# heheyas/V3D

Hardware: AMD Instinct MI355X
Metric: multi-view frames/sec, V3D_512 18-frame 25-step EDM (higher is better)
Workload: dtype bf16; 1 GPU; BASELINE.json configs[1]: V3D_512 random-init SVD-XT weights, 1x18x4x64x64 latent, 25 EulerEDM steps, cfg 4.5 (LinearPredictionGuider), 18-frame VideoDecoder decode to 512x512, one sample per GPU; frames=18, edm_steps=25, parallelism=replica x1, hip_graph=False

## Files before the change

include/v3d_hip.h:

```cpp
#ifndef V3D_HIP_H
#define V3D_HIP_H

#include <stdint.h>

#ifdef __cplusplus
extern "C" {
#endif

#define V3D_ABI_VERSION 9

typedef void* v3d_stream_t;

enum {
    V3D_OK = 0,
    V3D_ERR_ARG = -1,
    V3D_ERR_LAUNCH = -2,
};

int v3d_abi_version(void);
const char* v3d_last_error(void);
int v3d_device_info(int32_t* out4);

enum { V3D_GEMM_LINEAR = 0, V3D_GEMM_CONV3X3 = 1, V3D_GEMM_CONVT3 = 2 };

// ... 32 lines not shown
    const void* A2;
    int64_t K1, lda2;
} v3d_gemm_args;

int v3d_gemm(const v3d_gemm_args* args, v3d_stream_t stream);
int v3d_gemm_gn_in_supported(const v3d_gemm_args* args);

int v3d_ff_fused(const void* x, int64_t ldx, const void* W1p, const float* b1, const void* W2p, const float* b2,
                 const void* res1, int64_t ldr1, const void* res2, int64_t ldr2, const float* coef, int64_t coef_rpg,
                 float c_acc, float c_res1, float c_res2, void* out, int64_t ldo, int64_t M, int32_t C, int32_t hidden,
                 v3d_stream_t stream);

int v3d_ln_ff_fused(const void* x, int64_t ldx, float ln_eps, const void* W1p, const float* b1, const void* W2p, const float* b2,
                 const void* res1, int64_t ldr1, const void* res2, int64_t ldr2, const float* coef, int64_t coef_rpg,
                 float c_acc, float c_res1, float c_res2, void* out, int64_t ldo, int64_t M, int32_t C, int32_t hidden,
                 v3d_stream_t stream);
int v3d_ln_proj(const void* x, int64_t ldx, float eps, const void* Wp, const float* bias, void* out, int64_t ldo, void* outT,
                int64_t M, int32_t C, int32_t N, int32_t n_rm, int64_t S, v3d_stream_t stream);
int v3d_sizeof_gemm_args(void);

int v3d_groupnorm_stats(const void* x1, int64_t C1, const void* x2, int64_t C2, float* stats, int64_t nslots,
                        int64_t n_img, int64_t S, int32_t groups, int64_t imgs_per_stat, v3d_stream_t stream);
int v3d_groupnorm_stats_table(const void* x1, int64_t C1, const void* x2, int64_t C2, float* stats, int64_t nslots, uint32_t* tickets,
                              int64_t n_img, int64_t S, int32_t groups, int64_t imgs_per_stat, const float* gamma, const float* beta,
                              double count, float eps, float* table, v3d_stream_t stream);
int v3d_groupnorm_finalize(const float* stats, int64_t nslots, double* sums, int64_t n_stat, int32_t groups,
                           const float* gamma, const float* beta, int64_t C, double count, float eps, float* table,
                           v3d_stream_t stream);
int v3d_groupnorm_apply(const void* x1, int64_t C1, const void* x2, int64_t C2, const float* table, void* out,
                        int64_t n_img, int64_t S, int64_t imgs_per_stat, int32_t silu, v3d_stream_t stream);

// ... 103 lines not shown
```

v3d_amd/csrc/ff.hip:

```cpp
#include "common.h"

namespace {

struct FFP {
    const bf16_t* x;
    const bf16_t* W1;
    const bf16_t* W2;
    const float* b1;
    const float* b2;
    const bf16_t* res1;
    const bf16_t* res2;
    const float* coef;
    bf16_t* out;
    long long M, ldx, ldr1, ldr2, ldo, coef_rpg;
    float c_acc, c_res1, c_res2;
    int hidden;
    float ln_eps;
    unsigned w1_bytes, w2_bytes;
};

template <int I, int N, typename F>
__device__ __forceinline__ void ff_static_for(F&& f) {
    if constexpr (I < N) {
        f(std::integral_constant<int, I>{});
        ff_static_for<I + 1, N>(f);
    }
}

template <int NMFMA, int NVALU>
__device__ __forceinline__ void ff_tick_pipeline() {
    __builtin_amdgcn_sched_group_barrier(0x100, 8, 0);
    ff_static_for<0, NMFMA>([&](auto ic) __attribute__((always_inline)) {
        constexpr int i = decltype(ic)::value;
        __builtin_amdgcn_sched_group_barrier(0x008, 1, 0);
        __builtin_amdgcn_sched_group_barrier(0x100, 1, 0);
        if constexpr (i % 4 == 1) {
            __builtin_amdgcn_sched_group_barrier(0x004, 2, 0);
            __builtin_amdgcn_sched_group_barrier(0x020, 1, 0);
        }
        __builtin_amdgcn_sched_group_barrier(0x402, NVALU, 0);
    });
}

__device__ __forceinline__ int ff_swz(int row) { return (0x78 >> (((row >> 2) & 3) * 2)) & 3; }

template <int C, bool LN>
__global__ __launch_bounds__(256, 1) void ff_fused_kernel(FFP p) {
    constexpr int NT = C / 32;
    constexpr int NK = C / 16;
    constexpr int NO = C / 32;
    constexpr int W1_STAGE = 64 * 64;
    constexpr int W1_BYTES = NT * W1_STAGE;
    constexpr int W2_BYTES = C * 64;
    constexpr int NP1 = NT * 4, NP2 = C / 16;
    static_assert(NP1 % 4 == 0 && NP2 % 4 == 0, "pieces per wave");
    constexpr int PPW1 = NP1 / 4, PPW2 = NP2 / 4;
    constexpr int SROW = 128 + 16;
    constexpr int STAGE_REGION = 32 * SROW;
    static_assert(NO % 2 == 0, "staging geometry");
    constexpr int RING = 2 * W1_BYTES + 3 * W2_BYTES;
    constexpr int B2_OFF = RING + 4 * STAGE_REGION;
    constexpr int LDS_BYTES = B2_OFF + C * 4;
// ... 18 lines not shown
    const long long nblocks = p.M / 128;

    f32x16 acc2[NO];
#pragma unroll
    for (int o = 0; o < NO; ++o)
#pragma unroll
        for (int r = 0; r < 16; ++r) acc2[o][r] = 0.f;
    f32x16 sA[2][2];
    bf16x8 hh[2][2];
    bf16x8 xr[NK];

    auto load_x = [&](long long blk) __attribute__((always_inline)) {
        const bf16_t* xz = p.x + (blk * 128 + wave * 32 + l31) * p.ldx + hi * 8;
#pragma unroll
        for (int k = 0; k < NK; ++k) xr[k] = *reinterpret_cast<const bf16x8*>(xz + k * 16);
    };

    constexpr int NPD = 4;
    bf16x8 wf[NPD];
    int w2_wr_slot = 0, w2_rd_slot = 0;
    auto tick = [&](auto pa_c, auto pg_c, auto pb_c, auto pd_c, auto d2_c, int j) __attribute__((always_inline)) {
        constexpr int PA = decltype(pa_c)::value, PG = decltype(pg_c)::value, PB = decltype(pb_c)::value, PDM = decltype(pd_c)::value;
        constexpr bool D2 = decltype(d2_c)::value != 0;
        constexpr int NB = PB >= 0 ? 2 * NO : 0, NA = PA >= 0 ? 4 * NT : 0, NS = 2 * NO + 4 * NT;
        float4 bu[4], bv[4];
        const unsigned char* bz = reinterpret_cast<const unsigned char*>(p.b1 + (j == nslab ? 0 : j + 1) * 64 + hi * 4);
        if constexpr (PA >= 0) {
#pragma unroll
            for (int g = 0; g < 4; ++g) {
                bu[g] = *reinterpret_cast<const float4*>(bz + g * 32);
// ... 119 lines not shown
    ff_static_for<0, 2 * PPW1>([&](auto ic) __attribute__((always_inline)) {
        constexpr int k = decltype(ic)::value % PPW1, par = decltype(ic)::value / PPW1;
        __builtin_amdgcn_raw_ptr_buffer_load_lds(rsW1, (__attribute__((address_space(3))) void*)(w1ring + par * W1_BYTES + k * W1_STAGE + wave * 1024), 16,
                                                 (int)voff1, par * 64 * C * 2 + k * 4096, 0, 0);
    });
    ld1 = 2;
    ff_static_for<0, PPW2>([&](auto ic) __attribute__((always_inline)) {
        constexpr int k = decltype(ic)::value;
        __builtin_amdgcn_raw_ptr_buffer_load_lds(rsW2, (__attribute__((address_space(3))) void*)(w2ring + (wave + 4 * k) * 1024), 16, (int)voff2,
                                                 k * w2_step, 0, 0);
    });
    ld2 = 1;
    w2_wr_slot = 1;
    load_x(blk);
    asm volatile("s_waitcnt vmcnt(0)" ::: "memory");
    if constexpr (LN) ln_rows_inplace<NK>(xr, p.ln_eps);
    __builtin_amdgcn_s_barrier();
    tick(I0{}, IX{}, IX{}, IX{}, I0{}, -1);

    u32x4 r1[2][4];
    u32x2 r2[2][8];
    auto fetch_res = [&](long long mw0_, int ps, u32x4 (&q1)[4], u32x2 (&q2)[8]) __attribute__((always_inline)) {
        int lane_e = lane;
        asm volatile("" : "+v"(lane_e));
        if (p.res1) {
            const bf16_t* rz = p.res1 + mw0_ * p.ldr1 + ps * 64;
#pragma unroll
            for (int it = 0; it < 4; ++it) {
                const int c = it * 64 + lane_e;
                q1[it] = *reinterpret_cast<const u32x4*>(rz + (long long)(c >> 3) * p.ldr1 + (c & 7) * 8);
// ... 10 lines not shown
#pragma unroll
            for (int k = 0; k < 8; ++k) q2[k] = u32x2{0, 0};
        }
    };

    while (true) {
        const long long mw0 = blk * 128 + wave * 32;
        tick(I1{}, I0{}, IX{}, I0{}, I1{}, 0);
        for (int j = 1; j + 2 < nslab; j += 2) {
            tick(I0{}, I1{}, I0{}, I1{}, I1{}, j);
            tick(I1{}, I0{}, I1{}, I0{}, I1{}, j + 1);
        }
        const long long nxt = blk + gridDim.x;
        load_x(nxt < nblocks ? nxt : blk);
        tick(IX{}, I1{}, I0{}, I1{}, I0{}, nslab - 1);
        if constexpr (LN) ln_rows_inplace<NK>(xr, p.ln_eps);
        fetch_res(mw0, 0, r1[0], r2[0]);
        tick(I0{}, IX{}, I1{}, IX{}, I1{}, nslab);

        {
            int lane_e = lane;
            asm volatile("" : "+v"(lane_e));
            const int l31 = lane_e & 31, hi = lane_e >> 5, lane = lane_e;
            const long long m = mw0 + l31;
            float ca = p.c_acc, c1 = p.c_res1, c2 = p.c_res2;
            if (p.coef) {
                const float* cf = p.coef + (m / p.coef_rpg) * 3;
                ca = cf[0]; c1 = cf[1]; c2 = cf[2];
            }
#pragma unroll
            for (int ps = 0; ps < NO / 2; ++ps) {
                const int col0 = ps * 64;
                if (ps + 1 < NO / 2) fetch_res(mw0, ps + 1, r1[(ps + 1) & 1], r2[(ps + 1) & 1]);
                if (p.res1) {
#pragma unroll
                    for (int it = 0; it < 4; ++it) {
                        const int c = it * 64 + lane;
                        *reinterpret_cast<u32x4*>(stage + (c >> 3) * SROW + (c & 7) * 16) = r1[ps & 1][it];
                    }
                    asm volatile("s_waitcnt lgkmcnt(0)" ::: "memory");
                }
#pragma unroll
                for (int oo = 0; oo < 2; ++oo) {
                    const int o = ps * 2 + oo;
#pragma unroll
                    for (int g = 0; g < 4; ++g) {
                        const int ch = oo * 32 + g * 8 + hi * 4;
                        const float4 b = *reinterpret_cast<const float4*>(lds + B2_OFF + (col0 + ch) * 4);
                        float v[4] = {ca * (acc2[o][4 * g + 0] + b.x), ca * (acc2[o][4 * g + 1] + b.y), ca * (acc2[o][4 * g + 2] + b.z),
                                      ca * (acc2[o][4 * g + 3] + b.w)};
                        if (p.res1) {
                            const uint2 rr = *reinterpret_cast<const uint2*>(stage + l31 * SROW + ch * 2);
                            v[0] += c1 * bflo(rr.x); v[1] += c1 * bfhi(rr.x); v[2] += c1 * bflo(rr.y); v[3] += c1 * bfhi(rr.y);
                        }
                        if (p.res2) {
                            const u32x2 rr = r2[ps & 1][oo * 4 + g];
                            v[0] += c2 * bflo(rr.x); v[1] += c2 * bfhi(rr.x); v[2] += c2 * bflo(rr.y); v[3] += c2 * bfhi(rr.y);
                        }
                        *reinterpret_cast<uint2*>(stage + l31 * SROW + ch * 2) = make_uint2(pack2bf(v[0], v[1]), pack2bf(v[2], v[3]));
                    }
#pragma unroll
                    for (int r = 0; r < 16; ++r) acc2[o][r] = 0.f;
                }
                asm volatile("s_waitcnt lgkmcnt(0)" ::: "memory");
                bf16_t* oz = p.out + mw0 * p.ldo + col0;
#pragma unroll
                for (int c0 = 0; c0 < 256; c0 += 64) {
// ... 2 lines not shown
                        *reinterpret_cast<const uint4*>(stage + (c >> 3) * SROW + (c & 7) * 16);
                }
            }
        }
        if (nxt >= nblocks) break;
        blk = nxt;
    }
    asm volatile("s_waitcnt vmcnt(0)" ::: "memory");
}

}

static int ff_fused_launch(const void* x, int64_t ldx, float ln_eps, const void* W1p, const float* b1, const void* W2p, const float* b2,
                           const void* res1, int64_t ldr1, const void* res2, int64_t ldr2, const float* coef, int64_t coef_rpg,
                           float c_acc, float c_res1, float c_res2, void* out, int64_t ldo, int64_t M, int32_t C, int32_t hidden,
                           v3d_stream_t stream) {
    V3D_REQUIRE(x && W1p && b1 && W2p && b2 && out, "v3d_ff_fused: null pointer");
    V3D_REQUIRE(C == 320, "v3d_ff_fused: built for C = 320 (got %d); wider levels use the two-GEMM path", C);
    V3D_REQUIRE(hidden >= 128 && hidden % 64 == 0 && hidden * (long long)C * 4 < (1ll << 31), "v3d_ff_fused: bad hidden size %d", hidden);
    V3D_REQUIRE(M > 0 && M % 128 == 0, "v3d_ff_fused: M must be a multiple of 128 (got %lld)", (long long)M);
    V3D_REQUIRE(ldx % 8 == 0 && ldo % 8 == 0 && (!res1 || ldr1 % 8 == 0) && (!res2 || ldr2 % 4 == 0), "v3d_ff_fused: row strides");
    V3D_REQUIRE(((((uintptr_t)x | (uintptr_t)W1p | (uintptr_t)W2p | (uintptr_t)out | (uintptr_t)b1 | (uintptr_t)b2) & 15) == 0) &&
                    (!res1 || ((uintptr_t)res1 & 15) == 0) && (!res2 || ((uintptr_t)res2 & 7) == 0),
                "v3d_ff_fused: misaligned pointer");
    V3D_REQUIRE(!coef || coef_rpg > 0, "v3d_ff_fused: coef_rpg must be > 0");
    FFP p;
    p.x = (const bf16_t*)x; p.W1 = (const bf16_t*)W1p; p.W2 = (const bf16_t*)W2p; p.b1 = b1; p.b2 = b2;
    p.res1 = (const bf16_t*)res1; p.res2 = (const bf16_t*)res2; p.coef = coef; p.out = (bf16_t*)out;
    p.M = M; p.ldx = ldx; p.ldr1 = ldr1; p.ldr2 = ldr2; p.ldo = ldo; p.coef_rpg = coef_rpg;
    p.c_acc = c_acc; p.c_res1 = c_res1; p.c_res2 = c_res2; p.hidden = hidden; p.ln_eps = ln_eps;
    p.w1_bytes = (unsigned)(2ll * hidden * C * 2);
    p.w2_bytes = (unsigned)((long long)C * hidden * 2);
    const long long nblocks = M / 128;
    const int grid = (int)(nblocks < v3d_num_cus() ? nblocks : v3d_num_cus());
    if (ln_eps > 0.f)
        hipLaunchKernelGGL((ff_fused_kernel<320, true>), dim3(grid), dim3(256), 0, (hipStream_t)stream, p);
    else
        hipLaunchKernelGGL((ff_fused_kernel<320, false>), dim3(grid), dim3(256), 0, (hipStream_t)stream, p);
    return v3d_check_launch("v3d_ff_fused");
}

extern "C" int v3d_ff_fused(const void* x, int64_t ldx, const void* W1p, const float* b1, const void* W2p, const float* b2,
                            const void* res1, int64_t ldr1, const void* res2, int64_t ldr2, const float* coef, int64_t coef_rpg,
                            float c_acc, float c_res1, float c_res2, void* out, int64_t ldo, int64_t M, int32_t C, int32_t hidden,
                            v3d_stream_t stream) {
    return ff_fused_launch(x, ldx, 0.f, W1p, b1, W2p, b2, res1, ldr1, res2, ldr2, coef, coef_rpg, c_acc, c_res1, c_res2, out, ldo, M, C, hidden, stream);
}

extern "C" int v3d_ln_ff_fused(const void* x, int64_t ldx, float ln_eps, const void* W1p, const float* b1, const void* W2p, const float* b2,
                               const void* res1, int64_t ldr1, const void* res2, int64_t ldr2, const float* coef, int64_t coef_rpg,
                               float c_acc, float c_res1, float c_res2, void* out, int64_t ldo, int64_t M, int32_t C, int32_t hidden,
                               v3d_stream_t stream) {
    V3D_REQUIRE(ln_eps > 0.f, "v3d_ln_ff_fused: ln_eps must be > 0");
    return ff_fused_launch(x, ldx, ln_eps, W1p, b1, W2p, b2, res1, ldr1, res2, ldr2, coef, coef_rpg, c_acc, c_res1, c_res2, out, ldo, M, C, hidden, stream);
}
```

v3d_amd/csrc/norm.hip:

```cpp

#include "common.h"

namespace {

constexpr int NVMAX = 2;
constexpr int CMAX = 4096;

struct GNGeom {
    int VC;
    int TPR;
    int RPP;
    int NV;
};

__host__ __device__ inline GNGeom gn_geom(long long C) {
    GNGeom g;
    g.VC = (int)(C / 8);
    g.TPR = g.VC < 256 ? g.VC : 256;
    g.RPP = 256 / g.TPR;
    g.NV = (g.VC + g.TPR - 1) / g.TPR;
    return g;
}

__device__ __forceinline__ uint4 load_vec2(const bf16_t* x1, long long C1, const bf16_t* x2, long long C2, long long row, int c) {
// ... 171 lines not shown
            }
        }
#pragma unroll
        for (int j = 0; j < NV; ++j) {
            const int v = tcol + j * g.TPR;
            if (v < g.VC) {
#pragma unroll
                for (int e = 0; e < 8; ++e) {
                    sh_s[(long long)trow * C + v * 8 + e] = s[j][e];
                    sh_q[(long long)trow * C + v * 8 + e] = q[j][e];
                }
            }
        }
    }
    __syncthreads();
    const int cpg = (int)(C / groups);
    if (tid < groups) {
        float a = 0.f, b = 0.f;
        for (int r = 0; r < g.RPP; ++r)
            for (int c = tid * cpg; c < (tid + 1) * cpg; ++c) {
                a += sh_s[(long long)r * C + c];
                b += sh_q[(long long)r * C + c];
            }
        const long long slot = (img % imgs_per_stat) * gridDim.x + blockIdx.x;
        float* dst = stats + (((img / imgs_per_stat) * nslots + slot) * groups + tid) * 2;
        if constexpr (FUSE) {
            const f32x2_t v = {a, b};
            asm volatile("global_store_dwordx2 %0, %1, off sc0 sc1\n\ts_waitcnt vmcnt(0)" ::"v"(dst), "v"(v) : "memory");
        } else {
            dst[0] = a;
            dst[1] = b;
        }
    }
    if constexpr (FUSE) {
        __shared__ __attribute__((aligned(16))) unsigned ticket[4];
        const long long st = img / imgs_per_stat;
        const unsigned writers = (unsigned)(gridDim.x * imgs_per_stat);
        __syncthreads();
        if (tid == 0) ticket[0] = __hip_atomic_fetch_add(fz.tickets + st, 1u, __ATOMIC_RELAXED, __HIP_MEMORY_SCOPE_AGENT);
        __syncthreads();
        if (ticket[0] != writers - 1) return;
        gn_finalize_block<256, true>(reinterpret_cast<unsigned char*>(gn_sh), stats, nslots, (long long)writers, nullptr, groups, fz.gamma, fz.beta, C, fz.inv_count,
                                     fz.eps, fz.table, st);
        if (tid == 0) __hip_atomic_store(fz.tickets + st, 0u, __ATOMIC_RELAXED, __HIP_MEMORY_SCOPE_AGENT);
    }
}
// ... 191 lines not shown
}

}

namespace {
int gn_stats_launch(const char* who, const void* x1, int64_t C1, const void* x2, int64_t C2, float* stats, int64_t nslots, int64_t n_img, int64_t S,
                    int32_t groups, int64_t imgs_per_stat, const GNFuse* fz, v3d_stream_t stream) {
    int rc = gn_check(who, x1, C1, x2, C2, n_img, S, groups);
    if (rc) return rc;
    V3D_REQUIRE(stats != nullptr && imgs_per_stat > 0 && n_img % imgs_per_stat == 0, "%s: bad stats/imgs_per_stat", who);
    V3D_REQUIRE(nslots >= imgs_per_stat, "%s: nslots (%lld) must be >= imgs_per_stat (%lld): one slot per block", who,
                (long long)nslots, (long long)imgs_per_stat);
    const GNGeom g = gn_geom(C1 + C2);
    long long chunks, rpb;
    const long long bytes = n_img * S * (C1 + C2) * 2;
    gn_grid(n_img, S, g, chunks, rpb, bytes > (256ll << 20) ? 768 : 256);
    if (chunks * imgs_per_stat > nslots) {
        chunks = nslots / imgs_per_stat;
        rpb = (S + chunks - 1) / chunks;
        chunks = (S + rpb - 1) / rpb;
    }
    size_t shmem = (size_t)(C1 + C2) * 2 * g.RPP * sizeof(float);
    V3D_REQUIRE(shmem <= 64 * 1024, "%s: C=%lld needs %zu B of LDS", who, (long long)(C1 + C2), shmem);
    if (fz && shmem < (size_t)gn_fin_smem<256>()) shmem = (size_t)gn_fin_smem<256>();
    const dim3 grid((unsigned)chunks, (unsigned)n_img);
    const GNFuse none = {nullptr, nullptr, nullptr, nullptr, 0.0, 0.f};
    if (g.NV == 1) {
        if (fz)
            hipLaunchKernelGGL((gn_stats_kernel<1, 8, true>), grid, dim3(256), shmem, (hipStream_t)stream, (const bf16_t*)x1, (long long)C1,
                               (const bf16_t*)x2, (long long)C2, stats, (long long)nslots, (long long)S, groups, (long long)imgs_per_stat, rpb, *fz);
        else
// ... 50 lines not shown
    V3D_REQUIRE(table && out, "v3d_groupnorm_apply: null pointer");
    V3D_REQUIRE(((uintptr_t)table & 15) == 0, "v3d_groupnorm_apply: table must be 16-byte aligned");
    V3D_REQUIRE(imgs_per_stat > 0 && n_img % imgs_per_stat == 0, "v3d_groupnorm_apply: bad imgs_per_stat");
    const GNGeom g = gn_geom(C1 + C2);
    long long chunks, rpb;
    gn_grid(n_img, S, g, chunks, rpb);
    hipLaunchKernelGGL(gn_apply_kernel, dim3((unsigned)chunks, (unsigned)n_img), dim3(256), 0, (hipStream_t)stream,
                       (const bf16_t*)x1, (long long)C1, (const bf16_t*)x2, (long long)C2, table,
                       (bf16_t*)out, (long long)S, (long long)imgs_per_stat, silu, rpb);
    return v3d_check_launch("v3d_groupnorm_apply");
}

template <int NVT>
__global__ __launch_bounds__(256) void gn_small_kernel(const bf16_t* __restrict__ x1, long long C1, const bf16_t* __restrict__ x2, long long C2,
                                                       const float* __restrict__ gamma, const float* __restrict__ beta, bf16_t* __restrict__ out,
                                                       long long rows, int cpg, int GB, float eps, int silu) {
    extern __shared__ __attribute__((aligned(16))) unsigned char gn_small_lds[];
    float2* part = reinterpret_cast<float2*>(gn_small_lds);
    const int tid = threadIdx.x, lane = tid & 63, wave = tid >> 6;
    const long long C = C1 + C2;
    const int VB = GB * cpg / 8;
    const int vpg = cpg / 8;
    const long long row0 = (long long)blockIdx.y * rows;
    const int c0 = blockIdx.x * GB * cpg;
    const int NV = (int)rows * VB;
    float2* scsh = part + NV;
    float2* gstat = scsh + GB * cpg;
    uint4 v[NVT];
    const int dr = 256 / VB, dc = 256 - dr * VB;
    int r = tid / VB, vc = tid - r * VB;
    const int r_first = r, vc_first = vc;
#pragma unroll
    for (int k = 0; k < NVT; ++k) {
        const bool ok = tid + 256 * k < NV;
        v[k] = load_vec2(x1, C1, x2, C2, row0 + (ok ? r : 0), c0 + (ok ? vc : 0) * 8);
        r += dr; vc += dc;
        if (vc >= VB) { vc -= VB; ++r; }
    }
#pragma unroll
    for (int k = 0; k < NVT; ++k) {
        const int i = tid + 256 * k;
        if (i < NV) {
            float f[8];
            unpack8(v[k], f);
            float sm = 0.f, sq = 0.f;
#pragma unroll
            for (int e = 0; e < 8; ++e) { sm += f[e]; sq += f[e] * f[e]; }
            part[i] = make_float2(sm, sq);
        }
    }
    __syncthreads();
    for (int g = wave; g < GB; g += 4) {
        double sm = 0.0, sq = 0.0;
        for (int rr = lane; rr < (int)rows; rr += 64) {
            const float2* pr = part + rr * VB + g * vpg;
            for (int j = 0; j < vpg; ++j) {
                sm += (double)pr[j].x;
                sq += (double)pr[j].y;
            }
        }
#pragma unroll
        for (int o = 32; o >= 1; o >>= 1) {
            sm += __shfl_xor(sm, o, 64);
            sq += __shfl_xor(sq, o, 64);
        }
        if (lane == 0) {
            const double cnt = (double)rows * cpg;
            const double mean = sm / cnt;
            double var = sq / cnt - mean * mean;
            if (var < 0.0) var = 0.0;
            gstat[g] = make_float2((float)mean, (float)(1.0 / sqrt(var + (double)eps)));
        }
    }
    __syncthreads();
    for (int c = tid; c < GB * cpg; c += 256) {
        const float2 ms = gstat[c / cpg];
        const float sc = gamma[c0 + c] * ms.y;
        scsh[c] = make_float2(sc, beta[c0 + c] - ms.x * sc);
    }
    __syncthreads();
    r = r_first; vc = vc_first;
#pragma unroll
    for (int k = 0; k < NVT; ++k) {
        const int i = tid + 256 * k;
        if (i < NV) {
            float f[8];
            unpack8(v[k], f);
            const float4* t = reinterpret_cast<const float4*>(scsh + vc * 8);
#pragma unroll
            for (int e = 0; e < 8; e += 2) {
                const float4 q = t[e / 2];
                const float y0 = f[e] * q.x + q.y, y1 = f[e + 1] * q.z + q.w;
                f[e] = silu ? silu_f(y0) : y0;
                f[e + 1] = silu ? silu_f(y1) : y1;
            }
            *reinterpret_cast<uint4*>(out + (row0 + r) * C + c0 + vc * 8) = make_uint4(pack2bf(f[0], f[1]), pack2bf(f[2], f[3]), pack2bf(f[4], f[5]), pack2bf(f[6], f[7]));
        }
        r += dr; vc += dc;
        if (vc >= VB) { vc -= VB; ++r; }
    }
// ... 16 lines not shown
    return gn_small_groups(imgs_per_stat * S, C1, C2, groups) > 0;
}

extern "C" int v3d_groupnorm_small(const void* x1, int64_t C1, const void* x2, int64_t C2, const float* gamma, const float* beta, void* out,
                                   int64_t n_img, int64_t S, int32_t groups, int64_t imgs_per_stat, float eps, int32_t silu, v3d_stream_t stream) {
    int rc = gn_check("v3d_groupnorm_small", x1, C1, x2, C2, n_img, S, groups);
    if (rc) return rc;
    V3D_REQUIRE(gamma && beta && out, "v3d_groupnorm_small: null pointer");
    V3D_REQUIRE((((uintptr_t)gamma | (uintptr_t)beta | (uintptr_t)out) & 15) == 0, "v3d_groupnorm_small: gamma / beta / out must be 16-byte aligned");
    V3D_REQUIRE(imgs_per_stat > 0 && n_img % imgs_per_stat == 0, "v3d_groupnorm_small: bad imgs_per_stat");
    const long long rows = imgs_per_stat * S;
    const int gb = gn_small_groups(rows, C1, C2, groups);
    V3D_REQUIRE(gb > 0, "v3d_groupnorm_small: this tensor does not fit the one-launch form (v3d_groupnorm_small_supported)");
    const int cpg = (int)((C1 + C2) / 32);
    const long long nv = rows * (gb * cpg / 8);
    const size_t lds = (size_t)nv * 8 + (size_t)gb * cpg * 8 + 64;
    dim3 grid((unsigned)(32 / gb), (unsigned)(n_img / imgs_per_stat));
#define V3D_GNS_LAUNCH(NVT_)                                                                                                                    \
    hipLaunchKernelGGL((gn_small_kernel<NVT_>), grid, dim3(256), lds, (hipStream_t)stream, (const bf16_t*)x1, (long long)C1, (const bf16_t*)x2,     \
                       (long long)C2, gamma, beta, (bf16_t*)out, rows, cpg, gb, eps, silu)
    if (nv <= 256 * 8) V3D_GNS_LAUNCH(8);
    else if (nv <= 256 * 16) V3D_GNS_LAUNCH(16);
    else V3D_GNS_LAUNCH(24);
#undef V3D_GNS_LAUNCH
    return v3d_check_launch("v3d_groupnorm_small");
}

extern "C" int v3d_layernorm(const void* x, const float* add, int64_t add_rpg, int64_t add_ld, void* xsum_out,
                             const float* gamma, const float* beta, void* out, int64_t M, int64_t C, float eps,
                             v3d_stream_t stream) {
    V3D_REQUIRE(x && gamma && beta && out, "v3d_layernorm: null pointer");
    V3D_REQUIRE(C % 8 == 0 && C > 0 && C <= 64 * 8 * LNV, "v3d_layernorm: C=%lld unsupported (multiple of 8, <= %d)", (long long)C, 64 * 8 * LNV);
    V3D_REQUIRE(M > 0, "v3d_layernorm: bad M");
    V3D_REQUIRE(!add || add_rpg > 0, "v3d_layernorm: add_rpg must be > 0");
    V3D_REQUIRE(!xsum_out || add, "v3d_layernorm: xsum_out requires add");
// ... 22 lines not shown
```

v3d_amd/engine/packing.py:

```python
from __future__ import annotations

from dataclasses import dataclass, field
from typing import Dict, List, Optional

import torch
import torch.nn as nn

BF, F32 = torch.bfloat16, torch.float32


def _bf(t: torch.Tensor) -> torch.Tensor:
    from ..ops import get_ops
    return t.detach().to(get_ops().act_dtype).contiguous()


def _f(t: torch.Tensor) -> torch.Tensor:
    return t.detach().to(F32).contiguous()


def round_up(x: int, m: int) -> int:
    return (x + m - 1) // m * m


def pack_linear(lin: nn.Linear, k_pad: int = 0):
# ... 151 lines not shown
    proj_in: tuple
    proj_out: tuple
    s_norm1: tuple = None
    s_wqk: torch.Tensor = None
    s_wv: torch.Tensor = None
    s_wo: tuple = None
    s_ctx_off: int = 0
    s_norm3: tuple = None
    s_ff: FFPack = None
    t_norm_in: tuple = None
    t_ff_in: FFPack = None
    t_norm1: tuple = None
    t_wqkv: torch.Tensor = None
    s_wqkv_fused: Optional[tuple] = None
    t_wqkv_fused: Optional[tuple] = None
    t_wo: tuple = None
    t_ctx_off: int = 0
    s_attn2: object = None
    s_norm2: object = None
    t_attn2: object = None
    t_norm2: object = None
    x2: Dict = field(default_factory=dict)
    t_norm3: tuple = None
    t_ff: FFPack = None
    tpe: tuple = None
    max_period: float = 10000.0
    mixer: int = -1
    tables: Dict = field(default_factory=dict)


# ... 97 lines not shown
    assert st.d_head == 64, "attention kernels are specialised for d_head = 64"
    p.s_norm1 = pack_norm(blk.norm1)
    p.s_wqk = _bf(torch.cat([blk.attn1.to_q.weight.detach(), blk.attn1.to_k.weight.detach()], dim=0))
    p.s_wv = _bf(blk.attn1.to_v.weight)
    if C == 320:
        p.s_wqkv_fused = ln_proj_pack(torch.cat([blk.attn1.to_q.weight, blk.attn1.to_k.weight, blk.attn1.to_v.weight], dim=0), blk.norm1.weight, blk.norm1.bias)
        p.t_wqkv_fused = ln_proj_pack(torch.cat([tb.attn1.to_q.weight, tb.attn1.to_k.weight, tb.attn1.to_v.weight], dim=0), tb.norm1.weight, tb.norm1.bias)
    p.s_wo = pack_linear(blk.attn1.to_out[0])
    p.s_ctx_off = col.add_ctx(blk.attn2)
    p.s_attn2, p.s_norm2 = blk.attn2, blk.norm2
    p.s_norm3 = pack_norm(blk.norm3)
    p.s_ff = _pack_ff(blk.ff, blk.norm3)
    assert tb.ff_in is not False and tb.is_res
    p.t_norm_in = pack_norm(tb.norm_in)
    p.t_ff_in = _pack_ff(tb.ff_in)
    p.t_norm1 = pack_norm(tb.norm1)
    p.t_wqkv = _bf(torch.cat([tb.attn1.to_q.weight.detach(), tb.attn1.to_k.weight.detach(), tb.attn1.to_v.weight.detach()], dim=0))
    p.t_wo = pack_linear(tb.attn1.to_out[0])
    assert tb.attn2 is not None, "disable_temporal_crossattention is not used by V3D/SVD"
    p.t_ctx_off = col.add_ctx(tb.attn2)
    p.t_attn2, p.t_norm2 = tb.attn2, tb.norm2
    p.t_norm3 = pack_norm(tb.norm3)
    p.t_ff = _pack_ff(tb.ff, tb.norm3)
    p.tpe = pack_linear(st.time_pos_embed[0]) + pack_linear(st.time_pos_embed[2])
    p.max_period = float(st.max_time_embed_period)
    p.mixer = col.add_mixer(st.time_mixer, 1)
    return p


def cross_attn_pack(p: SVTPack, which: str):
# ... 169 lines not shown
```

v3d_amd/engine/unet.py:

```python
from __future__ import annotations

import os

from typing import Optional

import torch

from ..ops import GemmCall, get_ops
from .blocks import Env, Geo, unet_resblock
from .packing import SVTPack, UNetPack, cross_attn_pack, round_up

BF, F32 = torch.bfloat16, torch.float32


def _cast_rows_bf16(ops, x2d: torch.Tensor, pad_to: int = 0) -> torch.Tensor:
    n, C = x2d.shape
    return ops.nchw_to_nhwc_bf16(x2d.float().contiguous().reshape(n, C, 1), 1.0, max(pad_to, round_up(C, 8)))


def frame_pos_table(ops, p: SVTPack, B: int, frame_ids) -> torch.Tensor:
    key = (B, tuple(frame_ids))
    tab = p.tables.get(key)
    if tab is None:
        dev = p.proj_in[0].device
# ... 53 lines not shown
        v8, v_scale = ops.quant_fp8_slab(vT, p.heads)
        ops.attn_spatial_fp8(qk8, qk_scales, v8, v_scale, a, n, S, p.heads, 0.125)
    else:
        ops.attn_spatial(qk[:, :C], qk[:, C:], vT, a, n, S, p.heads, 0.125)
    multi = env.ctx_tok is not None
    if multi:
        x = ops.linear(a, p.s_wo[0], p.s_wo[1], res1=x)
        x = cross_attention(ops, x, cross_attn_pack(p, "s"), env.ctx_tok, env.n_ctx, p.heads)
    else:
        x = ops.linear(a, p.s_wo[0], p.s_wo[1], res1=x, add=ctx[:, p.s_ctx_off:], add_rpg=S, add_ld=ctx_ld)
    x_s = feed_forward(ops, x, p.s_ff, res1=x, ln=p.s_norm3)

    frames = range(T) if sh is None else sh.local_frames
    table = frame_pos_table(ops, p, B, frames)
    ga, be, eps = p.t_norm_in
    x_mix = ops.empty((n * S, C), ops.act_dtype, x.device)
    nin = ops.empty((n * S, C), ops.act_dtype, x.device)
    ops.layernorm(x_s, ga, be, nin, eps, add=table, add_rpg=S, add_ld=C, xsum_out=x_mix)
    x_t = feed_forward(ops, nin, p.t_ff_in, res1=x_mix)
    ga, be, eps = p.t_norm1
    ta = ops.empty((B, T, S, C), ops.act_dtype, x.device)
    if sh is None and ln_proj:
        qkv = ops.ln_proj(x_t, eps, p.t_wqkv_fused[0], p.t_wqkv_fused[1], 3 * C, S)[0].view(B, T, S, 3 * C)
        ops.attn_temporal(qkv[..., :C], qkv[..., C:2 * C], qkv[..., 2 * C:], ta, p.heads, 0.125)
    elif sh is None:
        n1 = ops.empty((n * S, C), ops.act_dtype, x.device) if n1 is None else n1
        ops.layernorm(x_t, ga, be, n1, eps)
        qkv = ops.linear(n1, p.t_wqkv).view(B, T, S, 3 * C)
        ops.attn_temporal(qkv[..., :C], qkv[..., C:2 * C], qkv[..., 2 * C:], ta, p.heads, 0.125)
    else:
        n1 = ops.empty((n * S, C), ops.act_dtype, x.device) if n1 is None else n1
        ops.layernorm(x_t, ga, be, n1, eps)
        kv_loc = ops.linear(n1, p.t_wqkv[C:]).view(B, T, S, 2 * C)
        kv, pending = sh.allgather_frames(kv_loc, async_op=True)
# ... 134 lines not shown
```

v3d_amd/hip.py:

```python
from __future__ import annotations

import ctypes as C
import os
from typing import Optional

import torch

from .ops import GemmCall, OpsBase

_HERE = os.path.dirname(os.path.abspath(__file__))
LIB_PATH = os.environ.get("V3D_HIP_LIB") or os.path.join(_HERE, "lib", "libv3d_hip.so")

ABI_VERSION = 9

c_i64, c_i32, c_f32, c_f64, c_vp = C.c_int64, C.c_int32, C.c_float, C.c_double, C.c_void_p


class _GemmArgs(C.Structure):
    _fields_ = [
        ("A", c_vp), ("W", c_vp), ("out", c_vp), ("bias", c_vp), ("add", c_vp), ("res1", c_vp), ("res2", c_vp),
        ("coef", c_vp),
        ("M", c_i64), ("N", c_i64), ("K", c_i64),
        ("lda", c_i64), ("ldw", c_i64), ("ldo", c_i64), ("ldr1", c_i64), ("ldr2", c_i64),
        ("a_rows", c_i64), ("a_row0", c_i64),
        ("add_rpg", c_i64), ("add_ld", c_i64), ("coef_rpg", c_i64),
        ("c_acc", c_f32), ("c_res1", c_f32), ("c_res2", c_f32),
        ("mode", c_i32), ("geglu", c_i32), ("out_fp32", c_i32),
        ("Hin", c_i32), ("Win", c_i32), ("Hout", c_i32), ("Wout", c_i32), ("stride", c_i32), ("up", c_i32),
# ... 13 lines not shown
    _fields_ = [("view", c_f32 * 16), ("proj", c_f32 * 16), ("tanfovx", c_f32), ("tanfovy", c_f32), ("bg", c_f32 * 3),
                ("width", c_i32), ("height", c_i32)]


_CAM = C.POINTER(GsCamera)

SIGNATURES = {
    "v3d_abi_version": (c_i32, []),
    "v3d_last_error": (C.c_char_p, []),
    "v3d_device_info": (c_i32, [c_vp]),
    "v3d_gemm": (c_i32, [C.POINTER(_GemmArgs), c_vp]),
    "v3d_sizeof_gemm_args": (c_i32, []),
    "v3d_ff_fused": (c_i32, [c_vp, c_i64, c_vp, c_vp, c_vp, c_vp, c_vp, c_i64, c_vp, c_i64, c_vp, c_i64, c_f32, c_f32, c_f32,
                             c_vp, c_i64, c_i64, c_i32, c_i32, c_vp]),
    "v3d_ln_ff_fused": (c_i32, [c_vp, c_i64, c_f32, c_vp, c_vp, c_vp, c_vp, c_vp, c_i64, c_vp, c_i64, c_vp, c_i64, c_f32, c_f32, c_f32,
                                c_vp, c_i64, c_i64, c_i32, c_i32, c_vp]),
    "v3d_ln_proj": (c_i32, [c_vp, c_i64, c_f32, c_vp, c_vp, c_vp, c_i64, c_vp, c_i64, c_i32, c_i32, c_i32, c_i64, c_vp]),
    "v3d_gemm_gn_in_supported": (c_i32, [C.POINTER(_GemmArgs)]),
    "v3d_groupnorm_stats": (c_i32, [c_vp, c_i64, c_vp, c_i64, c_vp, c_i64, c_i64, c_i64, c_i32, c_i64, c_vp]),
    "v3d_groupnorm_stats_table": (c_i32, [c_vp, c_i64, c_vp, c_i64, c_vp, c_i64, c_vp, c_i64, c_i64, c_i32, c_i64, c_vp, c_vp, C.c_double, C.c_float, c_vp, c_vp]),
    "v3d_groupnorm_finalize": (c_i32, [c_vp, c_i64, c_vp, c_i64, c_i32, c_vp, c_vp, c_i64, c_f64, c_f32, c_vp, c_vp]),
    "v3d_groupnorm_apply": (c_i32, [c_vp, c_i64, c_vp, c_i64, c_vp, c_vp, c_i64, c_i64, c_i64, c_i32, c_vp]),
    "v3d_groupnorm_small_supported": (c_i32, [c_i64, c_i64, c_i64, c_i32, c_i64]),
    "v3d_groupnorm_small": (c_i32, [c_vp, c_i64, c_vp, c_i64, c_vp, c_vp, c_vp, c_i64, c_i64, c_i32, c_i64, c_f32, c_i32, c_vp]),
    "v3d_layernorm": (c_i32, [c_vp, c_vp, c_i64, c_i64, c_vp, c_vp, c_vp, c_vp, c_i64, c_i64, c_f32, c_vp]),
    "v3d_attn_spatial": (c_i32, [c_vp, c_i64, c_vp, c_i64, c_vp, c_vp, c_i64, c_i64, c_i64, c_i32, c_f32, c_vp]),
    "v3d_attn_spatial_ld": (c_i32, [c_vp, c_i64, c_vp, c_i64, c_vp, c_i64, c_vp, c_i64, c_i64, c_i64, c_i32, c_f32, c_vp]),
    "v3d_attn_temporal": (c_i32, [c_vp, c_i64, c_i64, c_i64, c_vp, c_vp, c_i64, c_i64, c_i64, c_vp, c_i64, c_i64,
                                  c_i64, c_i64, c_i32, c_i32, c_i64, c_i32, c_f32, c_vp]),
    "v3d_attn_vae_d512": (c_i32, [c_vp, c_i64, c_vp, c_i64, c_vp, c_vp, c_vp, c_i64, c_i64, c_i64, c_i32, c_f32, c_vp]),
    "v3d_quant_fp8_tiles": (c_i32, [c_vp, c_i64, c_vp, c_i64, c_vp, c_i64, c_i64, c_i32, c_vp]),
# ... 481 lines not shown
        return out

    def ff_fused(self, x, w1p, b1, w2p, b2, out, *, res1=None, res2=None, coef=None, coef_rpg=0, c_acc=1.0, c_res1=1.0, c_res2=1.0):
        bf = torch.bfloat16
        for t, nm in ((x, "x"), (w1p, "w1"), (w2p, "w2"), (out, "out")):
            self._req(t, bf, f"ff.{nm}")
        M, Cc = x.shape
        hidden = w2p.shape[-1]
        self._check(self.lib.v3d_ff_fused(x.data_ptr(), x.stride(0), w1p.data_ptr(), b1.data_ptr(), w2p.data_ptr(), b2.data_ptr(),
                                          _ptr(res1), res1.stride(0) if res1 is not None else 0, _ptr(res2),
                                          res2.stride(0) if res2 is not None else 0, _ptr(coef), int(coef_rpg), float(c_acc),
                                          float(c_res1), float(c_res2), out.data_ptr(), out.stride(0), M, Cc, hidden, self._stream()),
                    "v3d_ff_fused")
        return out

    def ln_ff_fused(self, x, eps, w1p, b1, w2p, b2, out, *, res1=None, res2=None, coef=None, coef_rpg=0, c_acc=1.0, c_res1=1.0, c_res2=1.0):
        bf = torch.bfloat16
        for t, nm in ((x, "x"), (w1p, "w1"), (w2p, "w2"), (out, "out")):
            self._req(t, bf, f"ln_ff.{nm}")
        M, Cc = x.shape
        hidden = w2p.shape[-1]
        self._check(self.lib.v3d_ln_ff_fused(x.data_ptr(), x.stride(0), float(eps), w1p.data_ptr(), b1.data_ptr(), w2p.data_ptr(), b2.data_ptr(),
                                             _ptr(res1), res1.stride(0) if res1 is not None else 0, _ptr(res2),
                                             res2.stride(0) if res2 is not None else 0, _ptr(coef), int(coef_rpg), float(c_acc),
                                             float(c_res1), float(c_res2), out.data_ptr(), out.stride(0), M, Cc, hidden, self._stream()),
                    "v3d_ln_ff_fused")
        return out

    LN_PROJ_WIDTHS = (320,)

    def ln_proj(self, x, eps, wp, bias, n_rm, S):
        bf, f32 = torch.bfloat16, torch.float32
        self._req(x, bf, "ln_proj.x"); self._req_c(wp, bf, "ln_proj.w"); self._req_c(bias, f32, "ln_proj.bias")
        M, Cc = x.shape
        N = wp.shape[0]
        out = self.empty((M, n_rm), bf, x.device) if n_rm else None
        outT = self.empty((M // S, N - n_rm, S), bf, x.device) if n_rm < N else None
        self._check(self.lib.v3d_ln_proj(x.data_ptr(), x.stride(0), float(eps), wp.data_ptr(), bias.data_ptr(), _ptr(out),
                                         n_rm if out is not None else 0, _ptr(outT), M, Cc, N, n_rm, S, self._stream()), "v3d_ln_proj")
        return out, outT
# ... 238 lines not shown
```

Baseline: 12.74 frames/s.

## Fuse temporal pos-table add and LayerNorm into ff_in kernel; retune GroupNorm reductions

```diff
diff --git a/include/v3d_hip.h b/include/v3d_hip.h
--- a/include/v3d_hip.h
+++ b/include/v3d_hip.h
@@ -7,7 +7,7 @@
 extern "C" {
 #endif
 
-#define V3D_ABI_VERSION 9
+#define V3D_ABI_VERSION 10
 
 typedef void* v3d_stream_t;
 
@@ -70,7 +70,7 @@
 int v3d_ln_ff_fused(const void* x, int64_t ldx, float ln_eps, const void* W1p, const float* b1, const void* W2p, const float* b2,
                  const void* res1, int64_t ldr1, const void* res2, int64_t ldr2, const float* coef, int64_t coef_rpg,
                  float c_acc, float c_res1, float c_res2, void* out, int64_t ldo, int64_t M, int32_t C, int32_t hidden,
-                 v3d_stream_t stream);
+                 const float* add, int64_t add_rpg, int64_t add_ld, v3d_stream_t stream);
 int v3d_ln_proj(const void* x, int64_t ldx, float eps, const void* Wp, const float* bias, void* out, int64_t ldo, void* outT,
                 int64_t M, int32_t C, int32_t N, int32_t n_rm, int64_t S, v3d_stream_t stream);
 int v3d_sizeof_gemm_args(void);
diff --git a/v3d_amd/csrc/ff.hip b/v3d_amd/csrc/ff.hip
--- a/v3d_amd/csrc/ff.hip
+++ b/v3d_amd/csrc/ff.hip
@@ -16,6 +16,8 @@
     float c_acc, c_res1, c_res2;
     int hidden;
     float ln_eps;
+    const float* add;
+    long long add_rpg, add_ld;
     unsigned w1_bytes, w2_bytes;
 };
 
@@ -44,8 +46,9 @@
 
 __device__ __forceinline__ int ff_swz(int row) { return (0x78 >> (((row >> 2) & 3) * 2)) & 3; }
 
-template <int C, bool LN>
+template <int C, bool LN, bool ADD = false>
 __global__ __launch_bounds__(256, 1) void ff_fused_kernel(FFP p) {
+    static_assert(LN || !ADD, "the additive table belongs to the LayerNorm form");
     constexpr int NT = C / 32;
     constexpr int NK = C / 16;
     constexpr int NO = C / 32;
@@ -94,6 +97,21 @@
         const bf16_t* xz = p.x + (blk * 128 + wave * 32 + l31) * p.ldx + hi * 8;
 #pragma unroll
         for (int k = 0; k < NK; ++k) xr[k] = *reinterpret_cast<const bf16x8*>(xz + k * 16);
+    };
+    auto add_rows = [&](long long blk) __attribute__((always_inline)) {
+        const float* az = p.add + ((blk * 128 + wave * 32 + l31) / p.add_rpg) * p.add_ld + hi * 8;
+#pragma unroll
+        for (int k0 = 0; k0 < NK; k0 += 4) {
+#pragma unroll
+            for (int k = k0; k < k0 + 4; ++k) {
+                const float4 a0 = *reinterpret_cast<const float4*>(az + k * 16), a1 = *reinterpret_cast<const float4*>(az + k * 16 + 4);
+                const u32x4 u = __builtin_bit_cast(u32x4, xr[k]);
+                const u32x4 o = {pack2bf(bflo(u[0]) + a0.x, bfhi(u[0]) + a0.y), pack2bf(bflo(u[1]) + a0.z, bfhi(u[1]) + a0.w),
+                                 pack2bf(bflo(u[2]) + a1.x, bfhi(u[2]) + a1.y), pack2bf(bflo(u[3]) + a1.z, bfhi(u[3]) + a1.w)};
+                xr[k] = __builtin_bit_cast(bf16x8, o);
+            }
+            __builtin_amdgcn_sched_barrier(0);
+        }
     };
 
     constexpr int NPD = 4;
@@ -243,6 +261,7 @@
     w2_wr_slot = 1;
     load_x(blk);
     asm volatile("s_waitcnt vmcnt(0)" ::: "memory");
+    if constexpr (ADD) add_rows(blk);
     if constexpr (LN) ln_rows_inplace<NK>(xr, p.ln_eps);
     __builtin_amdgcn_s_barrier();
     tick(I0{}, IX{}, IX{}, IX{}, I0{}, -1);
@@ -283,6 +302,7 @@
         const long long nxt = blk + gridDim.x;
         load_x(nxt < nblocks ? nxt : blk);
         tick(IX{}, I1{}, I0{}, I1{}, I0{}, nslab - 1);
+        if constexpr (ADD) add_rows(nxt < nblocks ? nxt : blk);
         if constexpr (LN) ln_rows_inplace<NK>(xr, p.ln_eps);
         fetch_res(mw0, 0, r1[0], r2[0]);
         tick(I0{}, IX{}, I1{}, IX{}, I1{}, nslab);
@@ -301,6 +321,12 @@
             for (int ps = 0; ps < NO / 2; ++ps) {
                 const int col0 = ps * 64;
                 if (ps + 1 < NO / 2) fetch_res(mw0, ps + 1, r1[(ps + 1) & 1], r2[(ps + 1) & 1]);
+                [[maybe_unused]] float4 ad[8];
+                if constexpr (ADD) {
+                    const float* az = p.add + (m / p.add_rpg) * p.add_ld + col0 + hi * 4;
+#pragma unroll
+                    for (int q = 0; q < 8; ++q) ad[q] = *reinterpret_cast<const float4*>(az + (q >> 2) * 32 + (q & 3) * 8);
+                }
                 if (p.res1) {
 #pragma unroll
                     for (int it = 0; it < 4; ++it) {
@@ -319,7 +345,11 @@
                         float v[4] = {ca * (acc2[o][4 * g + 0] + b.x), ca * (acc2[o][4 * g + 1] + b.y), ca * (acc2[o][4 * g + 2] + b.z),
                                       ca * (acc2[o][4 * g + 3] + b.w)};
                         if (p.res1) {
-                            const uint2 rr = *reinterpret_cast<const uint2*>(stage + l31 * SROW + ch * 2);
+                            uint2 rr = *reinterpret_cast<const uint2*>(stage + l31 * SROW + ch * 2);
+                            if constexpr (ADD) {
+                                const float4 a = ad[oo * 4 + g];
+                                rr = make_uint2(pack2bf(bflo(rr.x) + a.x, bfhi(rr.x) + a.y), pack2bf(bflo(rr.y) + a.z, bfhi(rr.y) + a.w));
+                            }
                             v[0] += c1 * bflo(rr.x); v[1] += c1 * bfhi(rr.x); v[2] += c1 * bflo(rr.y); v[3] += c1 * bfhi(rr.y);
                         }
                         if (p.res2) {
@@ -352,7 +382,7 @@
 static int ff_fused_launch(const void* x, int64_t ldx, float ln_eps, const void* W1p, const float* b1, const void* W2p, const float* b2,
                            const void* res1, int64_t ldr1, const void* res2, int64_t ldr2, const float* coef, int64_t coef_rpg,
                            float c_acc, float c_res1, float c_res2, void* out, int64_t ldo, int64_t M, int32_t C, int32_t hidden,
-                           v3d_stream_t stream) {
+                           const float* add, int64_t add_rpg, int64_t add_ld, v3d_stream_t stream) {
     V3D_REQUIRE(x && W1p && b1 && W2p && b2 && out, "v3d_ff_fused: null pointer");
     V3D_REQUIRE(C == 320, "v3d_ff_fused: built for C = 320 (got %d); wider levels use the two-GEMM path", C);
     V3D_REQUIRE(hidden >= 128 && hidden % 64 == 0 && hidden * (long long)C * 4 < (1ll << 31), "v3d_ff_fused: bad hidden size %d", hidden);
@@ -362,16 +392,21 @@
                     (!res1 || ((uintptr_t)res1 & 15) == 0) && (!res2 || ((uintptr_t)res2 & 7) == 0),
                 "v3d_ff_fused: misaligned pointer");
     V3D_REQUIRE(!coef || coef_rpg > 0, "v3d_ff_fused: coef_rpg must be > 0");
+    V3D_REQUIRE(!add || (ln_eps > 0.f && res1 && add_rpg > 0 && add_ld % 4 == 0 && ((uintptr_t)add & 15) == 0),
+                "v3d_ln_ff_fused: add needs res1, add_rpg > 0, add_ld %% 4 == 0 and a 16-byte aligned table");
     FFP p;
     p.x = (const bf16_t*)x; p.W1 = (const bf16_t*)W1p; p.W2 = (const bf16_t*)W2p; p.b1 = b1; p.b2 = b2;
     p.res1 = (const bf16_t*)res1; p.res2 = (const bf16_t*)res2; p.coef = coef; p.out = (bf16_t*)out;
     p.M = M; p.ldx = ldx; p.ldr1 = ldr1; p.ldr2 = ldr2; p.ldo = ldo; p.coef_rpg = coef_rpg;
     p.c_acc = c_acc; p.c_res1 = c_res1; p.c_res2 = c_res2; p.hidden = hidden; p.ln_eps = ln_eps;
+    p.add = add; p.add_rpg = add_rpg; p.add_ld = add_ld;
     p.w1_bytes = (unsigned)(2ll * hidden * C * 2);
     p.w2_bytes = (unsigned)((long long)C * hidden * 2);
     const long long nblocks = M / 128;
     const int grid = (int)(nblocks < v3d_num_cus() ? nblocks : v3d_num_cus());
-    if (ln_eps > 0.f)
+    if (add)
+        hipLaunchKernelGGL((ff_fused_kernel<320, true, true>), dim3(grid), dim3(256), 0, (hipStream_t)stream, p);
+    else if (ln_eps > 0.f)
         hipLaunchKernelGGL((ff_fused_kernel<320, true>), dim3(grid), dim3(256), 0, (hipStream_t)stream, p);
     else
         hipLaunchKernelGGL((ff_fused_kernel<320, false>), dim3(grid), dim3(256), 0, (hipStream_t)stream, p);
@@ -382,13 +417,15 @@
                             const void* res1, int64_t ldr1, const void* res2, int64_t ldr2, const float* coef, int64_t coef_rpg,
                             float c_acc, float c_res1, float c_res2, void* out, int64_t ldo, int64_t M, int32_t C, int32_t hidden,
                             v3d_stream_t stream) {
-    return ff_fused_launch(x, ldx, 0.f, W1p, b1, W2p, b2, res1, ldr1, res2, ldr2, coef, coef_rpg, c_acc, c_res1, c_res2, out, ldo, M, C, hidden, stream);
+    return ff_fused_launch(x, ldx, 0.f, W1p, b1, W2p, b2, res1, ldr1, res2, ldr2, coef, coef_rpg, c_acc, c_res1, c_res2, out, ldo, M, C, hidden, nullptr, 0, 0,
+                           stream);
 }
 
 extern "C" int v3d_ln_ff_fused(const void* x, int64_t ldx, float ln_eps, const void* W1p, const float* b1, const void* W2p, const float* b2,
                                const void* res1, int64_t ldr1, const void* res2, int64_t ldr2, const float* coef, int64_t coef_rpg,
                                float c_acc, float c_res1, float c_res2, void* out, int64_t ldo, int64_t M, int32_t C, int32_t hidden,
-                               v3d_stream_t stream) {
+                               const float* add, int64_t add_rpg, int64_t add_ld, v3d_stream_t stream) {
     V3D_REQUIRE(ln_eps > 0.f, "v3d_ln_ff_fused: ln_eps must be > 0");
-    return ff_fused_launch(x, ldx, ln_eps, W1p, b1, W2p, b2, res1, ldr1, res2, ldr2, coef, coef_rpg, c_acc, c_res1, c_res2, out, ldo, M, C, hidden, stream);
-}
+    return ff_fused_launch(x, ldx, ln_eps, W1p, b1, W2p, b2, res1, ldr1, res2, ldr2, coef, coef_rpg, c_acc, c_res1, c_res2, out, ldo, M, C, hidden, add, add_rpg,
+                           add_ld, stream);
+}
diff --git a/v3d_amd/csrc/norm.hip b/v3d_amd/csrc/norm.hip
--- a/v3d_amd/csrc/norm.hip
+++ b/v3d_amd/csrc/norm.hip
@@ -209,22 +209,37 @@
         }
     }
     __syncthreads();
-    const int cpg = (int)(C / groups);
-    if (tid < groups) {
-        float a = 0.f, b = 0.f;
-        for (int r = 0; r < g.RPP; ++r)
-            for (int c = tid * cpg; c < (tid + 1) * cpg; ++c) {
+    if (g.RPP > 1) {
+        for (int c = tid; c < (int)C; c += 256) {
+            float a = sh_s[c], b = sh_q[c];
+            for (int r = 1; r < g.RPP; ++r) {
                 a += sh_s[(long long)r * C + c];
                 b += sh_q[(long long)r * C + c];
             }
-        const long long slot = (img % imgs_per_stat) * gridDim.x + blockIdx.x;
-        float* dst = stats + (((img / imgs_per_stat) * nslots + slot) * groups + tid) * 2;
-        if constexpr (FUSE) {
-            const f32x2_t v = {a, b};
-            asm volatile("global_store_dwordx2 %0, %1, off sc0 sc1\n\ts_waitcnt vmcnt(0)" ::"v"(dst), "v"(v) : "memory");
-        } else {
-            dst[0] = a;
-            dst[1] = b;
+            sh_s[c] = a;
+            sh_q[c] = b;
+        }
+        __syncthreads();
+    }
+    const int cpg = (int)(C / groups);
+    for (int t = tid; t < groups * 8; t += 256) {
+        const int gi = t >> 3, q = t & 3;
+        const float* src = ((t & 4) ? sh_q : sh_s) + gi * cpg;
+        float a = 0.f;
+        for (int c = (q * cpg) >> 2; c < ((q + 1) * cpg) >> 2; ++c) a += src[c];
+        a += __shfl_xor(a, 1, 64);
+        a += __shfl_xor(a, 2, 64);
+        const float b = __shfl_down(a, 4, 64);
+        if ((t & 7) == 0) {
+            const long long slot = (img % imgs_per_stat) * gridDim.x + blockIdx.x;
+            float* dst = stats + (((img / imgs_per_stat) * nslots + slot) * groups + gi) * 2;
+            if constexpr (FUSE) {
+                const f32x2_t v = {a, b};
+                asm volatile("global_store_dwordx2 %0, %1, off sc0 sc1\n\ts_waitcnt vmcnt(0)" ::"v"(dst), "v"(v) : "memory");
+            } else {
+                dst[0] = a;
+                dst[1] = b;
+            }
         }
     }
     if constexpr (FUSE) {
@@ -446,7 +461,7 @@
     const GNGeom g = gn_geom(C1 + C2);
     long long chunks, rpb;
     const long long bytes = n_img * S * (C1 + C2) * 2;
-    gn_grid(n_img, S, g, chunks, rpb, bytes > (256ll << 20) ? 768 : 256);
+    gn_grid(n_img, S, g, chunks, rpb, bytes > (256ll << 20) ? 768 : (bytes >= (64ll << 20) ? 512 : 256));
     if (chunks * imgs_per_stat > nslots) {
         chunks = nslots / imgs_per_stat;
         rpb = (S + chunks - 1) / chunks;
@@ -527,7 +542,7 @@
 template <int NVT>
 __global__ __launch_bounds__(256) void gn_small_kernel(const bf16_t* __restrict__ x1, long long C1, const bf16_t* __restrict__ x2, long long C2,
                                                        const float* __restrict__ gamma, const float* __restrict__ beta, bf16_t* __restrict__ out,
-                                                       long long rows, int cpg, int GB, float eps, int silu) {
+                                                       long long rows, int cpg, int GB, int rps, float eps, int silu) {
     extern __shared__ __attribute__((aligned(16))) unsigned char gn_small_lds[];
     float2* part = reinterpret_cast<float2*>(gn_small_lds);
     const int tid = threadIdx.x, lane = tid & 63, wave = tid >> 6;
@@ -535,10 +550,14 @@
     const int VB = GB * cpg / 8;
     const int vpg = cpg / 8;
     const long long row0 = (long long)blockIdx.y * rows;
-    const int c0 = blockIdx.x * GB * cpg;
+    const int gsh = __ffs(GB) - 1;
+    const int split = blockIdx.x >> (5 - gsh);
+    const int c0 = (blockIdx.x & ((32 >> gsh) - 1)) * GB * cpg;
+    const int r_lo = split * rps, r_hi = r_lo + rps;
     const int NV = (int)rows * VB;
     float2* scsh = part + NV;
     float2* gstat = scsh + GB * cpg;
+    double* upart = reinterpret_cast<double*>(gstat + 8);
     uint4 v[NVT];
     const int dr = 256 / VB, dc = 256 - dr * VB;
     int r = tid / VB, vc = tid - r * VB;
@@ -563,9 +582,19 @@
         }
     }
     __syncthreads();
-    for (int g = wave; g < GB; g += 4) {
+    const int bands = ((int)rows + 63) / 64;
+    const int RS = GB >= 4 || bands < 2 ? 1 : (4 / GB < bands ? 4 / GB : bands), NU = GB * RS;
+    const double cnt = (double)rows * cpg;
+    auto finish = [&](int g, double sm, double sq) __attribute__((always_inline)) {
+        const double mean = sm / cnt;
+        double var = sq / cnt - mean * mean;
+        if (var < 0.0) var = 0.0;
+        gstat[g] = make_float2((float)mean, (float)(1.0 / sqrt(var + (double)eps)));
+    };
+    for (int u = wave; u < NU; u += 4) {
+        const int g = u & (GB - 1), rs = u >> gsh;
         double sm = 0.0, sq = 0.0;
-        for (int rr = lane; rr < (int)rows; rr += 64) {
+        for (int rr = rs * 64 + lane; rr < (int)rows; rr += 64 * RS) {
             const float2* pr = part + rr * VB + g * vpg;
             for (int j = 0; j < vpg; ++j) {
                 sm += (double)pr[j].x;
@@ -578,11 +607,23 @@
             sq += __shfl_xor(sq, o, 64);
         }
         if (lane == 0) {
-            const double cnt = (double)rows * cpg;
-            const double mean = sm / cnt;
-            double var = sq / cnt - mean * mean;
-            if (var < 0.0) var = 0.0;
-            gstat[g] = make_float2((float)mean, (float)(1.0 / sqrt(var + (double)eps)));
+            if (RS == 1) {
+                finish(g, sm, sq);
+            } else {
+                upart[u * 2] = sm;
+                upart[u * 2 + 1] = sq;
+            }
+        }
+    }
+    if (RS > 1) {
+        __syncthreads();
+        if (tid < GB) {
+            double sm = upart[tid * 2], sq = upart[tid * 2 + 1];
+            for (int rs = 1; rs < RS; ++rs) {
+                sm += upart[(rs * GB + tid) * 2];
+                sq += upart[(rs * GB + tid) * 2 + 1];
+            }
+            finish(tid, sm, sq);
         }
     }
     __syncthreads();
@@ -596,7 +637,7 @@
 #pragma unroll
     for (int k = 0; k < NVT; ++k) {
         const int i = tid + 256 * k;
-        if (i < NV) {
+        if (i < NV && r >= r_lo && r < r_hi) {
             float f[8];
             unpack8(v[k], f);
             const float4* t = reinterpret_cast<const float4*>(scsh + vc * 8);
@@ -643,11 +684,16 @@
     V3D_REQUIRE(gb > 0, "v3d_groupnorm_small: this tensor does not fit the one-launch form (v3d_groupnorm_small_supported)");
     const int cpg = (int)((C1 + C2) / 32);
     const long long nv = rows * (gb * cpg / 8);
-    const size_t lds = (size_t)nv * 8 + (size_t)gb * cpg * 8 + 64;
-    dim3 grid((unsigned)(32 / gb), (unsigned)(n_img / imgs_per_stat));
+    const size_t lds = (size_t)nv * 8 + (size_t)gb * cpg * 8 + 64 + 128;
+    const int nslice = 32 / gb;
+    const long long n_stat = n_img / imgs_per_stat;
+    int ns = 1;
+    while (ns < 8 && nslice * n_stat * ns * 2 <= v3d_num_cus() && rows >= 32 * ns) ns *= 2;
+    const int rps = (int)((rows + ns - 1) / ns);
+    dim3 grid((unsigned)(nslice * ns), (unsigned)n_stat);
 #define V3D_GNS_LAUNCH(NVT_)                                                                                                                    \
     hipLaunchKernelGGL((gn_small_kernel<NVT_>), grid, dim3(256), lds, (hipStream_t)stream, (const bf16_t*)x1, (long long)C1, (const bf16_t*)x2,     \
-                       (long long)C2, gamma, beta, (bf16_t*)out, rows, cpg, gb, eps, silu)
+                       (long long)C2, gamma, beta, (bf16_t*)out, rows, cpg, gb, rps, eps, silu)
     if (nv <= 256 * 8) V3D_GNS_LAUNCH(8);
     else if (nv <= 256 * 16) V3D_GNS_LAUNCH(16);
     else V3D_GNS_LAUNCH(24);
diff --git a/v3d_amd/engine/packing.py b/v3d_amd/engine/packing.py
--- a/v3d_amd/engine/packing.py
+++ b/v3d_amd/engine/packing.py
@@ -189,6 +189,7 @@
     t_wqkv: torch.Tensor = None
     s_wqkv_fused: Optional[tuple] = None
     t_wqkv_fused: Optional[tuple] = None
+    t_ff_in_ln: Optional[tuple] = None
     t_wo: tuple = None
     t_ctx_off: int = 0
     s_attn2: object = None
@@ -316,6 +317,10 @@
     assert tb.ff_in is not False and tb.is_res
     p.t_norm_in = pack_norm(tb.norm_in)
     p.t_ff_in = _pack_ff(tb.ff_in)
+    if p.t_ff_in.w2_fused is not None:
+        lin1, lin2 = tb.ff_in.net[0].proj, tb.ff_in.net[2]
+        w1p, b1p, _ = ff_fused_pack(lin1.weight.detach(), lin1.bias.detach(), lin2.weight.detach(), ln=(tb.norm_in.weight, tb.norm_in.bias))
+        p.t_ff_in_ln = (w1p, b1p, float(tb.norm_in.eps))
     p.t_norm1 = pack_norm(tb.norm1)
     p.t_wqkv = _bf(torch.cat([tb.attn1.to_q.weight.detach(), tb.attn1.to_k.weight.detach(), tb.attn1.to_v.weight.detach()], dim=0))
     p.t_wo = pack_linear(tb.attn1.to_out[0])
diff --git a/v3d_amd/engine/unet.py b/v3d_amd/engine/unet.py
--- a/v3d_amd/engine/unet.py
+++ b/v3d_amd/engine/unet.py
@@ -91,10 +91,16 @@
     frames = range(T) if sh is None else sh.local_frames
     table = frame_pos_table(ops, p, B, frames)
     ga, be, eps = p.t_norm_in
-    x_mix = ops.empty((n * S, C), ops.act_dtype, x.device)
-    nin = ops.empty((n * S, C), ops.act_dtype, x.device)
-    ops.layernorm(x_s, ga, be, nin, eps, add=table, add_rpg=S, add_ld=C, xsum_out=x_mix)
-    x_t = feed_forward(ops, nin, p.t_ff_in, res1=x_mix)
+    ff = p.t_ff_in
+    if _FF_FUSED and _LN_FF and p.t_ff_in_ln is not None and (n * S) % 128 == 0 and getattr(ops, "LN_FF_ADD", False):
+        w1_ln, b1_ln, ln_eps = p.t_ff_in_ln
+        x_t = ops.ln_ff_fused(x_s, ln_eps, w1_ln, b1_ln, ff.w2_fused, ff.b2, ops.empty((n * S, C), ops.act_dtype, x.device),
+                              res1=x_s, add=table, add_rpg=S, add_ld=C)
+    else:
+        x_mix = ops.empty((n * S, C), ops.act_dtype, x.device)
+        nin = ops.empty((n * S, C), ops.act_dtype, x.device)
+        ops.layernorm(x_s, ga, be, nin, eps, add=table, add_rpg=S, add_ld=C, xsum_out=x_mix)
+        x_t = feed_forward(ops, nin, ff, res1=x_mix)
     ga, be, eps = p.t_norm1
     ta = ops.empty((B, T, S, C), ops.act_dtype, x.device)
     if sh is None and ln_proj:
diff --git a/v3d_amd/hip.py b/v3d_amd/hip.py
--- a/v3d_amd/hip.py
+++ b/v3d_amd/hip.py
@@ -11,7 +11,7 @@
 _HERE = os.path.dirname(os.path.abspath(__file__))
 LIB_PATH = os.environ.get("V3D_HIP_LIB") or os.path.join(_HERE, "lib", "libv3d_hip.so")
 
-ABI_VERSION = 9
+ABI_VERSION = 10
 
 c_i64, c_i32, c_f32, c_f64, c_vp = C.c_int64, C.c_int32, C.c_float, C.c_double, C.c_void_p
 
@@ -55,7 +55,7 @@
     "v3d_ff_fused": (c_i32, [c_vp, c_i64, c_vp, c_vp, c_vp, c_vp, c_vp, c_i64, c_vp, c_i64, c_vp, c_i64, c_f32, c_f32, c_f32,
                              c_vp, c_i64, c_i64, c_i32, c_i32, c_vp]),
     "v3d_ln_ff_fused": (c_i32, [c_vp, c_i64, c_f32, c_vp, c_vp, c_vp, c_vp, c_vp, c_i64, c_vp, c_i64, c_vp, c_i64, c_f32, c_f32, c_f32,
-                                c_vp, c_i64, c_i64, c_i32, c_i32, c_vp]),
+                                c_vp, c_i64, c_i64, c_i32, c_i32, c_vp, c_i64, c_i64, c_vp]),
     "v3d_ln_proj": (c_i32, [c_vp, c_i64, c_f32, c_vp, c_vp, c_vp, c_i64, c_vp, c_i64, c_i32, c_i32, c_i32, c_i64, c_vp]),
     "v3d_gemm_gn_in_supported": (c_i32, [C.POINTER(_GemmArgs)]),
     "v3d_groupnorm_stats": (c_i32, [c_vp, c_i64, c_vp, c_i64, c_vp, c_i64, c_i64, c_i64, c_i32, c_i64, c_vp]),
@@ -567,16 +567,22 @@
                     "v3d_ff_fused")
         return out
 
-    def ln_ff_fused(self, x, eps, w1p, b1, w2p, b2, out, *, res1=None, res2=None, coef=None, coef_rpg=0, c_acc=1.0, c_res1=1.0, c_res2=1.0):
+    LN_FF_ADD = True
+
+    def ln_ff_fused(self, x, eps, w1p, b1, w2p, b2, out, *, res1=None, res2=None, coef=None, coef_rpg=0, c_acc=1.0, c_res1=1.0, c_res2=1.0,
+                    add=None, add_rpg=0, add_ld=0):
         bf = torch.bfloat16
         for t, nm in ((x, "x"), (w1p, "w1"), (w2p, "w2"), (out, "out")):
             self._req(t, bf, f"ln_ff.{nm}")
+        if add is not None:
+            self._req(add, torch.float32, "ln_ff.add")
         M, Cc = x.shape
         hidden = w2p.shape[-1]
         self._check(self.lib.v3d_ln_ff_fused(x.data_ptr(), x.stride(0), float(eps), w1p.data_ptr(), b1.data_ptr(), w2p.data_ptr(), b2.data_ptr(),
                                              _ptr(res1), res1.stride(0) if res1 is not None else 0, _ptr(res2),
                                              res2.stride(0) if res2 is not None else 0, _ptr(coef), int(coef_rpg), float(c_acc),
-                                             float(c_res1), float(c_res2), out.data_ptr(), out.stride(0), M, Cc, hidden, self._stream()),
+                                             float(c_res1), float(c_res2), out.data_ptr(), out.stride(0), M, Cc, hidden,
+                                             _ptr(add), int(add_rpg), int(add_ld), self._stream()),
                     "v3d_ln_ff_fused")
         return out
 
```

After: 12.82 frames/s, median of 6. About the same (+0.6%).
